# lambdaclass/lambdaworks_kzg

Hardware: NVIDIA B200
Metric: blobs/sec commit+proof (higher is better)
Workload: dtype u32 (12x32-bit Montgomery limbs, IMAD.WIDE)

## Files before the change

### lambdaworks_kzg_b200/csrc/kernels.h

```cpp
#pragma once
#include <cuda_runtime.h>
#include <stddef.h>
#include <stdint.h>

#define LW_SAME_CARVEOUT(kernel)                                                                              \
  do {                                                                                                        \
    static bool lw_done_[64] = {};                                                                            \
    int lw_dev_ = 0;                                                                                          \
    if (cudaGetDevice(&lw_dev_) == cudaSuccess && lw_dev_ >= 0 && lw_dev_ < 64 && !lw_done_[lw_dev_]) {       \
      cudaFuncSetAttribute(kernel, cudaFuncAttributePreferredSharedMemoryCarveout, cudaSharedmemCarveoutMaxShared); \
      lw_done_[lw_dev_] = true;                                                                               \
    }                                                                                                         \
  } while (0)

namespace lw {

constexpr int N_POINTS = 4096;
constexpr int BLOB_BYTES = 4096 * 32;
constexpr int AFFINE_BYTES = 96;
constexpr int XYZZ_BYTES = 192;

uint64_t launches();
void count_launch(int n = 1);

void launch_srs_import(void* d_aff_out, const void* d_canon_in, int* d_not_on_curve, int* d_not_in_subgroup, int n, cudaStream_t st);
void launch_table_bases(void* d_bases, const void* d_aff, int c, int nwin, int npoints, cudaStream_t st);
void launch_table_fill(void* d_table, const void* d_bases, int c, int nwin, int npoints, uint32_t cnt_top, cudaStream_t st);
int table_num_windows(int c);
uint32_t table_top_count(int c);
unsigned long long table_entries(int c, int npoints);

void launch_msm_gather(void* d_partials, const void* d_table, int c, const void* d_scalars, bool be_input,
                       int n_blobs, int blocks_per_blob, cudaStream_t st);
void launch_msm_gather_ba(void* d_partials, const void* d_table, int c, const void* d_scalars, bool be_input,
                          int n_blobs, void* d_scratch, cudaStream_t st, int split = 1);
size_t msm_ba_scratch_bytes(int n_blobs);
int msm_ba_threads();
int msm_ba_slots();
int msm_ba_num_variants();
void msm_ba_set_variant(int v);
void launch_msm_finalize(void* d_out48, void* d_aff_out, const void* d_partials, int parts_per_blob, int n_blobs, cudaStream_t st);
int msm_threads_per_block();

void launch_challenge_midstate(void* d_states, const void* d_blobs, int n, cudaStream_t st, bool latency = false, bool be_header = false);
void launch_challenge_finish(void* d_z, const void* d_states, const void* d_blobs, const void* d_commit48, int n, cudaStream_t st, bool le_digest = false);
void launch_fr_from_be(void* d_z, const void* d_z_be32, int n, cudaStream_t st);
void launch_poly_eval_quot(void* d_q, void* d_y, void* d_y_be32, const void* d_blobs, const void* d_z, int n, cudaStream_t st);

void launch_g1_decompress(void* d_aff, void* d_recompressed48, int* d_status, const void* d_in48, int n, cudaStream_t st, bool strict = false,
                          bool check_subgroup = true);
void launch_g1_subgroup_check(int* d_status, const void* d_aff, int n, cudaStream_t st, bool strict = false);
void launch_status_or(int* d_status, const int* d_other, int n, cudaStream_t st);
void launch_zero_failed(void* d_out, int bytes_per_item, const int* d_status, int n, cudaStream_t st);

void launch_synth_blobs(void* d_blobs, uint64_t first_blob, size_t n, cudaStream_t st);
double run_imad_peak(int variant);

struct G2PreparedDev;
size_t g2_prepared_bytes();
void launch_g2_prepare(void* d_prepared, int* d_bad, const void* d_canon_in, cudaStream_t st);
void launch_g2_check(int* d_bad, const void* d_canon_in, int n, cudaStream_t st);
void launch_verify_single(int* d_ok, const void* d_c_aff, const void* d_pi_aff, const void* d_z, const void* d_y,
                          const void* d_g1_0_aff, const void* d_prep0, const void* d_prep1, bool g1_0_in_subgroup, cudaStream_t st,
                          int* d_status = nullptr, int sub_code = 0);
void launch_make_tuples(void* d_tuples160, const void* d_c48, const void* d_z, const void* d_y, const void* d_pi48, int n, cudaStream_t st, bool le = false);
void launch_batch_challenge(void* d_r, const void* d_tuples160, size_t n_total, cudaStream_t st, int wire = 0);
size_t batch_challenge_state_bytes();
int batch_challenge_blocks_ready(size_t tuples_ready);
void launch_batch_challenge_part(void* d_r, void* d_state, const void* d_tuples160, size_t n_total, int blk0, int blk1, bool first, bool last,
                                 cudaStream_t st, int wire = 0);
void launch_batch_partials(void* d_partial288, const void* d_r, const void* d_c_aff, const void* d_pi_aff, const void* d_z, const void* d_y,
                           size_t first, int n_local, void* d_scratch, cudaStream_t st, cudaStream_t st2, cudaEvent_t ev_fork, cudaEvent_t ev_join);
size_t batch_partials_scratch_bytes(int n_local);
void launch_batch_final(int* d_ok, const void* d_partials288, int n_ranks, const void* d_prep0, const void* d_prep1, cudaStream_t st);
void launch_batch_final_each(int* d_ok, const void* d_partials288, int n_checks, const void* d_prep0, const void* d_prep1, cudaStream_t st);

void launch_write_generator(void* d_out, cudaStream_t st);
void launch_le_roots(void* d_roots, cudaStream_t st);
void launch_le_idft_rows(void* d_rows, cudaStream_t st);
void launch_affine_to_canon(void* d_out24, const void* d_aff, int n, cudaStream_t st);
void launch_le_blob_check(int* d_status, const void* d_blobs, int n, cudaStream_t st, bool be = false);
void launch_le_fr_parse(void* d_out, int* d_status, const void* d_in32, int n, cudaStream_t st, bool be = false);
void launch_le_eval_quot(void* d_q, void* d_y, void* d_y_le32, const void* d_blobs, const void* d_z, const void* d_roots, int n, cudaStream_t st,
                         bool be = false);

void launch_var_msm(void* d_out48, const void* d_points_xy_be, const void* d_scalars_be, size_t n, void* d_scratch, cudaStream_t st,
                    bool points_in_g1 = false);
void launch_var_msm_mont(void* d_out_affine_be96, const void* d_points_mont, const void* d_scalars_canon8, size_t n, void* d_scratch, cudaStream_t st);
size_t var_msm_scratch_bytes(size_t n);
size_t var_msm_bad_flag_offset(size_t n, bool points_in_g1 = false);
int var_msm_window_bits(size_t n);
void launch_var_msm_synth(void* d_pts_be, void* d_sc_be, const void* d_table, unsigned long long n_entries, unsigned long long seed, size_t n,
                          cudaStream_t st);

}
```

### lambdaworks_kzg_b200/csrc/lwkzg.cu

```cuda
#include <cuda_runtime.h>
#include <fcntl.h>
#include <signal.h>
#include <sys/file.h>
#include <unistd.h>

#include <algorithm>
#include <atomic>
#include <condition_variable>
#include <chrono>
#include <cstdio>
#include <cstdlib>
#include <cstring>
#include <map>
#include <mutex>
#include <string>
#include <thread>
#include <vector>

#include "../../include/lwkzg.h"
#include "kernels.h"
#include "kernels_cells.h"
#include "kernels_setup.h"

namespace {
// ... 548 lines not shown
  c->mode = mode;
  c->c = c->nwin = 0;
  c->srs_valid = c->srs_in_g1 = c->g2_valid = false;
  c->g1_host = g1;
  c->g2_host = g2;
  if (!build_ctx_inner(c, g1, g2, mode, window_override)) {
    std::string e = tl_err;
    destroy_ctx(c);
    set_err(e);
    return nullptr;
  }
  return c;
}

struct LazyKey {
  const void* g1;
  const void* g2;
  uint64_t hash;
  bool operator<(const LazyKey& o) const {
    if (g1 != o.g1) return g1 < o.g1;
    if (g2 != o.g2) return g2 < o.g2;
    return hash < o.hash;
  }
};
std::map<LazyKey, Ctx*>& lazy_map() {
  static std::map<LazyKey, Ctx*> m;
  return m;
}
uint64_t fnv1a(const void* p, size_t n, uint64_t h) {
  const uint64_t* w = (const uint64_t*)p;
  for (size_t i = 0; i < n / 8; i++) {
    h ^= w[i];
    h *= 1099511628211ull;
  }
  return h;
}

std::mutex g_lazy_mu;

void destroy_ctx_locked(Ctx* c) {
  if (!c) return;
  { std::lock_guard<std::mutex> lk(c->mu); }
  destroy_ctx(c);
}

Ctx* ctx_of(const KZGSettings* s) {
  if (!s || !s->g1_values || !s->g2_values) {
    set_err("null KZGSettings");
    return nullptr;
  }
  if (s->fs) {
    Ctx* c = reinterpret_cast<Ctx*>(s->fs);
    if (c->magic == CTX_MAGIC) return c;
  }
  LazyKey key{s->g1_values, s->g2_values, 0};
  key.hash = fnv1a(s->g1_values, sizeof(g1_t) * N_POINTS);
  key.hash = fnv1a(s->g2_values, sizeof(g2_t) * 2, key.hash);
  std::lock_guard<std::mutex> lk(g_lazy_mu);
  auto it = lazy_map().find(key);
  if (it != lazy_map().end()) return it->second;
  for (auto j = lazy_map().begin(); j != lazy_map().end();) {
    if (j->first.g1 == key.g1 && j->first.g2 == key.g2) {
      destroy_ctx_locked(j->second);
      j = lazy_map().erase(j);
    } else {
      ++j;
    }
  }
  Ctx* c = build_ctx(s->g1_values, s->g2_values);
  if (c) lazy_map()[key] = c;
  return c;
}

enum class Mode { Commit, CommitProve, BlobProof, PointProof };

bool use_batch_affine(int n) {
  std::lock_guard<std::mutex> lk(g_mu);
  return opts().msm_algo == 1 && n >= opts().msm_ba_min_blobs;
}

size_t chunk_at(size_t off, size_t n, size_t chunk) { return std::min(chunk, n - off); }

int ba_block_slots() {
  static int slots[64] = {};
  int dev = 0;
  if (cudaGetDevice(&dev) != cudaSuccess || dev < 0 || dev >= 64) return 444;
  if (!slots[dev]) {
    int sms = 148;
    cudaDeviceGetAttribute(&sms, cudaDevAttrMultiProcessorCount, dev);
    slots[dev] = 3 * sms;
  }
  return slots[dev];
}

int auto_bpb(int n) {
  if (use_batch_affine(n)) {
    int split = 1;
    while (split < 8 && n * split * 2 <= ba_block_slots()) split *= 2;
    return split;
  }
  long o;
  {
    std::lock_guard<std::mutex> lk(g_mu);
    o = opts().msm_blocks_per_blob;
  }
  if (o > 0) return (int)o;
  int target = (1024 + n - 1) / n;
  int b = 1;
  while (b < target) b <<= 1;
  return std::min(b, 128);
}

void run_msm(Slot& s, const Ctx* c, const void* d_scalars, bool be_input, int n, int bpb, cudaStream_t st);

BufList slot_buffers(Slot& s, int n, int bpb, bool need_blobs) {
  const size_t m = (size_t)n;
  BufList bufs;
  if (use_batch_affine(n)) bufs.push_back({&s.ba_scratch, msm_ba_scratch_bytes(n * bpb)});
  if (need_blobs) bufs.push_back({&s.blobs, m * BLOB_BYTES});
  bufs.insert(bufs.end(), {{&s.q, m * BLOB_BYTES}, {&s.partials, m * bpb * XYZZ_BYTES}, {&s.states, m * 32}, {&s.z, m * 32}, {&s.y, m * 32},
                           {&s.ybe, m * 32}, {&s.c48, m * 48}, {&s.cin48, m * 48}, {&s.p48, m * 48}, {&s.caff, m * AFFINE_BYTES},
                           {&s.status, m * sizeof(int)}, {&s.status2, m * sizeof(int)}, {&s.zbe, m * 32}});
  return bufs;
}

void run_msm(Slot& s, const Ctx* c, const void* d_scalars, bool be_input, int n, int bpb, cudaStream_t st) {
  if (bpb <= 8 && use_batch_affine(n) && s.ba_scratch.cap >= msm_ba_scratch_bytes(n * bpb))
    launch_msm_gather_ba(s.partials.p, c->d_table, c->c, d_scalars, be_input, n, s.ba_scratch.p, st, bpb);
  else
    launch_msm_gather(s.partials.p, c->d_table, c->c, d_scalars, be_input, n, bpb, st);
}

bool enqueue_chunk(Ctx* c, Slot& s, Mode mode, const void* d_blobs, int n, void* d_c48, void* d_p48, void* d_ybe, int* d_status,
                   const void* d_commit_in48, const void* d_z_in_be) {
  const int bpb = auto_bpb(n);
  cudaStream_t st = s.st;
  const bool le = c->lagrange();
  if (le) {
    const bool be = c->be_wire();
    int* stt = d_status ? d_status : (int*)s.status.p;
    CU_TRY(cudaMemsetAsync(stt, 0, (size_t)n * sizeof(int), st));
    launch_le_blob_check(stt, d_blobs, n, st, be);
    if (mode == Mode::Commit) {
      run_msm(s, c, d_blobs, be, n, bpb, st);
      launch_msm_finalize(d_c48, nullptr, s.partials.p, bpb, n, st);
      return true;
    }
    const void* commit_for_hash = nullptr;
    if (mode == Mode::CommitProve || mode == Mode::BlobProof) {
      CU_TRY(cudaEventRecord(s.ev_fork, st));
      CU_TRY(cudaStreamWaitEvent(s.aux, s.ev_fork, 0));
      launch_challenge_midstate(s.states.p, d_blobs, n, s.aux, mode == Mode::BlobProof, be);
      CU_TRY(cudaEventRecord(s.ev_aux, s.aux));
    }
    if (mode == Mode::CommitProve) {
      run_msm(s, c, d_blobs, be, n, bpb, st);
      launch_msm_finalize(d_c48, nullptr, s.partials.p, bpb, n, st);
      commit_for_hash = d_c48;
    } else if (mode == Mode::BlobProof) {
      launch_g1_decompress(nullptr, nullptr, (int*)s.status2.p, d_commit_in48, n, st, true);
      launch_status_or(stt, (const int*)s.status2.p, n, st);
      commit_for_hash = d_commit_in48;
    }
    if (mode == Mode::PointProof) {
      CU_TRY(cudaMemsetAsync(s.status2.p, 0, (size_t)n * sizeof(int), st));
      launch_le_fr_parse(s.z.p, (int*)s.status2.p, d_z_in_be, n, st, be);
      launch_status_or(stt, (const int*)s.status2.p, n, st);
    } else {
      CU_TRY(cudaStreamWaitEvent(st, s.ev_aux, 0));
      launch_challenge_finish(s.z.p, s.states.p, d_blobs, commit_for_hash, n, st, !be);
    }
    launch_le_eval_quot(s.q.p, nullptr, d_ybe, d_blobs, s.z.p, c->d_roots, n, st, be);
    run_msm(s, c, s.q.p, false, n, bpb, st);
    launch_msm_finalize(d_p48, nullptr, s.partials.p, bpb, n, st);
    return true;
// ... 588 lines not shown

bool first_bad_status(Ctx* c, size_t n, int& code) {
  std::vector<int> st(n);
  CU_TRY(cudaMemcpy(st.data(), c->vb_status.p, n * sizeof(int), cudaMemcpyDeviceToHost));
  code = 0;
  for (int v : st)
    if (v) { code = v; break; }
  return true;
}
C_KZG_RET bad_code(int code) { return code == 1 ? C_KZG_BADARGS : C_KZG_ERROR; }

bool verify_single_from_workspace(Ctx* c, bool& ok, bool deferred_subgroup = false, int* bad = nullptr) {
  cudaStream_t s0 = c->slot[0].st;
  launch_verify_single((int*)c->vb_ok.p, c->vb_caff.p, c->vb_piaff.p, c->vb_z.p, c->vb_y.p, c->lagrange() ? c->d_gen : c->d_srs, c->d_prep0, c->d_prep1,
                       c->lagrange() || c->srs_in_g1, s0, deferred_subgroup ? (int*)c->vb_status.p : nullptr, c->lagrange() ? 1 : 2);
  int out[2] = {0, 0};
  CU_TRY(cudaMemcpyAsync(&out[0], c->vb_ok.p, sizeof(int), cudaMemcpyDeviceToHost, s0));
  if (deferred_subgroup) CU_TRY(cudaMemcpyAsync(&out[1], c->vb_status.p, sizeof(int), cudaMemcpyDeviceToHost, s0));
  CU_TRY(cudaStreamSynchronize(s0));
  CU_TRY(cudaGetLastError());
  ok = out[0] != 0;
  if (bad) *bad = out[1];
  return true;
}

struct CtxLock {
  Ctx* c;
  std::unique_lock<std::mutex> lk;
  DeviceGuard dg;
  explicit CtxLock(Ctx* ctx) : c(ctx), lk(ctx->mu), dg(ctx->device) {}
};

#include "cells_host.inl"

}

extern "C" {

const char* lwkzg_last_error(void) { return tl_err.c_str(); }
const char* lwkzg_version(void) { return "lwkzg-b200 0.2 (sm_100a)"; }
uint64_t lwkzg_kernel_launches(void) { return lw::launches(); }

int lwkzg_set_option(const char* name, long value) {
  std::lock_guard<std::mutex> lk(g_mu);
  std::string n(name ? name : "");
  if (n == "window_bits") { if (value < 4 || value > 16) return 1; opts().window_bits = value; return 0; }
  if (n == "msm_blocks_per_blob") { if (value < 0 || value > 256 || (value > 64 && (value & (value - 1)))) return 1; opts().msm_blocks_per_blob = value; return 0; }
  if (n == "chunk_blobs") { if (value < 1 || value > (1 << 20)) return 1; opts().chunk_blobs = value; return 0; }
  if (n == "mode") { if (value < 0 || value > 2) return 1; opts().mode = value; return 0; }
  if (n == "msm_algo") { if (value != 0 && value != 1) return 1; opts().msm_algo = value; return 0; }
  if (n == "msm_ba_min_blobs") { if (value < 1) return 1; opts().msm_ba_min_blobs = value; return 0; }
  if (n == "verify_super_blobs") { if (value < 1) return 1; opts().verify_super_blobs = value; return 0; }
  if (n == "lincomb_points_in_g1") { if (value != 0 && value != 1) return 1; opts().lincomb_points_in_g1 = value; return 0; }
  if (n == "share_table") { if (value != 0 && value != 1) return 1; opts().share_table = value; return 0; }
  if (n == "verify_streams") { if (value < 1 || value > 8) return 1; opts().verify_streams = value; return 0; }
  if (n == "verify_split_subgroup") { if (value != 0 && value != 1) return 1; opts().verify_split_subgroup = value; return 0; }
  if (n == "cache_config") { if (value < 0 || value > 3) return 1; opts().cache_config = value; return 0; }
  if (n == "verify_overlap_decode") { if (value != 0 && value != 1) return 1; opts().verify_overlap_decode = value; return 0; }
  if (n == "cell_window_bits") { if (value < 4 || value > 14) return 1; opts().cell_window_bits = value; return 0; }
  if (n == "cell_chunk_blobs") { if (value < 1 || value > 65536) return 1; opts().cell_chunk_blobs = value; return 0; }
  if (n == "msm_ba_variant") { if (value < 0 || value >= msm_ba_num_variants()) return 1; msm_ba_set_variant((int)value); return 0; }
  return 1;
}
long lwkzg_get_option(const char* name) {
  std::lock_guard<std::mutex> lk(g_mu);
  std::string n(name ? name : "");
  if (n == "window_bits") return opts().window_bits;
  if (n == "msm_blocks_per_blob") return opts().msm_blocks_per_blob;
  if (n == "chunk_blobs") return opts().chunk_blobs;
  if (n == "mode") return opts().mode;
  if (n == "msm_algo") return opts().msm_algo;
  if (n == "msm_ba_min_blobs") return opts().msm_ba_min_blobs;
  if (n == "verify_super_blobs") return opts().verify_super_blobs;
  if (n == "lincomb_points_in_g1") return opts().lincomb_points_in_g1;
  if (n == "share_table") return opts().share_table;
  if (n == "verify_streams") return opts().verify_streams;
  if (n == "verify_split_subgroup") return opts().verify_split_subgroup;
  if (n == "cache_config") return opts().cache_config;
  if (n == "verify_overlap_decode") return opts().verify_overlap_decode;
  if (n == "cell_window_bits") return opts().cell_window_bits;
  if (n == "cell_chunk_blobs") return opts().cell_chunk_blobs;
  if (n == "msm_ba_threads") return msm_ba_threads();
  if (n == "msm_ba_slots") return msm_ba_slots();
  return -1;
}

double lwkzg_imad_peak(int variant) { return lw::run_imad_peak(variant); }

C_KZG_RET load_trusted_setup(KZGSettings* out, const uint8_t* g1_bytes, size_t n1, const uint8_t* g2_bytes, size_t n2) {
  if (n1 != TRUSTED_SETUP_NUM_G1_POINTS || n2 != TRUSTED_SETUP_NUM_G2_POINTS) return C_KZG_BADARGS;
  if (!out || !g1_bytes || !g2_bytes) return C_KZG_ERROR;
  return settings_from_compressed(out, g1_bytes, n1, g2_bytes, n2);
}

C_KZG_RET load_trusted_setup_file(KZGSettings* out, FILE* in) {
  if (!out || !in) return C_KZG_ERROR;
  std::string contents;
  char buf[65536];
  size_t got;
  while ((got = fread(buf, 1, sizeof(buf), in)) > 0) contents.append(buf, got);
  std::vector<std::string> lines;
  size_t pos = 0;
  while (pos < contents.size()) {
    size_t nl = contents.find('\n', pos);
    std::string ln = contents.substr(pos, nl == std::string::npos ? std::string::npos : nl - pos);
    if (!ln.empty() && ln.back() == '\r') ln.pop_back();
    lines.push_back(ln);
    if (nl == std::string::npos) break;
    pos = nl + 1;
  }
  size_t n1 = 0, n2 = 0;
  if (lines.size() < 2 || !parse_usize(lines[0], n1) || !parse_usize(lines[1], n2)) { set_err("invalid trusted setup header"); return C_KZG_ERROR; }
  if (n1 > (1u << 20) || n2 > (1u << 20)) { set_err("implausible point counts"); return C_KZG_ERROR; }
  size_t avail = lines.size() - 2;
  size_t m1 = std::min(n1, avail), m2 = std::min(n2, avail - m1);
  std::vector<uint8_t> g1b(m1 * 48 + 1), g2b(m2 * 96 + 1);
  for (size_t i = 0; i < m1; i++)
    if (!hex_line(lines[2 + i], &g1b[i * 48], 48)) { set_err("bad G1 hex line"); return C_KZG_ERROR; }
  for (size_t i = 0; i < m2; i++)
    if (!hex_line(lines[2 + m1 + i], &g2b[i * 96], 96)) { set_err("bad G2 hex line"); return C_KZG_ERROR; }
  return settings_from_compressed(out, g1b.data(), m1, g2b.data(), m2);
}

C_KZG_RET free_trusted_setup(KZGSettings* s) {
  if (!s) return C_KZG_OK;
  if (s->fs) {
    Ctx* c = reinterpret_cast<Ctx*>(s->fs);
    if (c->magic == CTX_MAGIC) destroy_ctx_locked(c);
    s->fs = nullptr;
  } else {
    std::lock_guard<std::mutex> lk(g_lazy_mu);
    for (auto j = lazy_map().begin(); j != lazy_map().end();) {
      if (j->first.g1 == s->g1_values && j->first.g2 == s->g2_values) {
        destroy_ctx_locked(j->second);
        j = lazy_map().erase(j);
      } else {
        ++j;
      }
    }
  }
  free(s->g1_values);
  free(s->g2_values);
  s->g1_values = nullptr;
  s->g2_values = nullptr;
  return C_KZG_OK;
}

C_KZG_RET lwkzg_blob_to_kzg_commitment_batch(KZGCommitment* out, const Blob* blobs, size_t n, const KZGSettings* s, int* status) {
  return host_batch(Mode::Commit, s, n, blobs, nullptr, nullptr, out, nullptr, nullptr, status);
}
C_KZG_RET lwkzg_compute_blob_kzg_proof_batch(KZGProof* out, const Blob* blobs, const Bytes48* commitments, size_t n, const KZGSettings* s, int* status) {
  return host_batch(Mode::BlobProof, s, n, blobs, commitments, nullptr, nullptr, out, nullptr, status);
}
C_KZG_RET lwkzg_compute_kzg_proof_batch(KZGProof* proofs, Bytes32* ys, const Blob* blobs, const Bytes32* zs, size_t n, const KZGSettings* s, int* status) {
  return host_batch(Mode::PointProof, s, n, blobs, nullptr, zs, nullptr, proofs, ys, status);
}
C_KZG_RET lwkzg_commit_and_prove_batch(KZGCommitment* commitments, KZGProof* proofs, const Blob* blobs, size_t n, const KZGSettings* s, int* status) {
  return host_batch(Mode::CommitProve, s, n, blobs, nullptr, nullptr, commitments, proofs, nullptr, status);
}

C_KZG_RET lwkzg_commit_and_prove_batch_device(void* d_commitments, void* d_proofs, const void* d_blobs, size_t n, const KZGSettings* s, void* stream, void* d_status) {
  return device_batch(Mode::CommitProve, s, n, d_blobs, nullptr, d_commitments, d_proofs, d_status, (cudaStream_t)stream);
}
C_KZG_RET lwkzg_blob_to_kzg_commitment_batch_device(void* d_commitments, const void* d_blobs, size_t n, const KZGSettings* s, void* stream, void* d_status) {
  return device_batch(Mode::Commit, s, n, d_blobs, nullptr, d_commitments, nullptr, d_status, (cudaStream_t)stream);
}
// ... 446 lines not shown
```

### lambdaworks_kzg_b200/csrc/msm.cu

```cuda
#include "msm_common.cuh"

namespace lw {

int msm_threads_per_block() { return MSM_THREADS; }

template <bool BE>
__global__ void __launch_bounds__(MSM_THREADS, LWKZG_MSM_MIN_BLOCKS)
msm_gather_kernel(G1Xyzz* __restrict__ partials, const uint4* __restrict__ table, const uint8_t* __restrict__ scalars,
                  int c, int nwin, uint32_t cnt_top, int pt_threads, int wsplit) {
  constexpr int HT = MSM_THREADS / 2;
  __shared__ uint32_t sk[4][MSM_THREADS];
  __shared__ uint32_t red[48 * HT];

  const int tid = threadIdx.x;
  const int half = tid / HT;
  const int blob = blockIdx.y;
  const int q = blockIdx.x * HT + (tid % HT);
  const int pl = q % pt_threads;
  const int wg = q / pt_threads;
  const uint8_t* sc = scalars + (size_t)blob * BLOB_BYTES;
  auto limb = [&](int w) { return sk[w][tid]; };

  G1Xyzz acc = xyzz_inf();

  for (int pi = pl; pi < N_POINTS; pi += pt_threads) {
    uint32_t h4[4];
    load_scalar_half<BE>(h4, sc, pi, half);
#pragma unroll
    for (int i = 0; i < 4; i++) sk[i][tid] = h4[i];
    int carry = 0;
    int d = 0;
    G1Affine cur = g1a_inf();
    for (int j = 0; j <= nwin; j++) {
      int dn = 0;
      G1Affine nxt = g1a_inf();
      if (j < nwin) {
        dn = glv_digit(limb, c, nwin, j, carry);
        if ((j % wsplit) != wg) dn = 0;
        if (dn != 0) nxt = load_entry(table, entry_index(c, nwin, cnt_top, j, pi, dn < 0 ? -dn : dn));
      }
      if (d != 0) {
        cur.y = fp_cneg(cur.y, d < 0);
        xyzz_madd_hot(acc, cur);
      }
      cur = nxt; d = dn;
    }
  }

  block_reduce_xyzz_glv<MSM_THREADS>(acc, red);
  if (tid == 0) partials[(size_t)blob * gridDim.x + blockIdx.x] = acc;
}

void launch_msm_gather(void* d_partials, const void* d_table, int c, const void* d_scalars, bool be_input, int n_blobs,
                       int blocks_per_blob, cudaStream_t st);
#define LW_BA_DECL(N) void launch_ba_v##N(void*, const void*, int, const void*, bool, int, void*, cudaStream_t, int)
LW_BA_DECL(0); LW_BA_DECL(1);
struct BaVariant { int k, threads; };
static const BaVariant BA_VARIANTS[] = {{64, 128}, {64, 64}};
constexpr int N_BA_VARIANTS = (int)(sizeof(BA_VARIANTS) / sizeof(BA_VARIANTS[0]));
static int g_ba_variant = 0;
void msm_ba_set_variant(int v) { if (v >= 0 && v < N_BA_VARIANTS) g_ba_variant = v; }
int msm_ba_num_variants() { return N_BA_VARIANTS; }
int msm_ba_threads() { return BA_VARIANTS[g_ba_variant].threads; }
int msm_ba_slots() { return BA_VARIANTS[g_ba_variant].k; }
size_t msm_ba_scratch_bytes(int n_blobs) {
  return (size_t)n_blobs * 64 * 9 * 128 * sizeof(uint4);
}

void launch_msm_gather_ba(void* d_partials, const void* d_table, int c, const void* d_scalars, bool be_input, int n_blobs,
                          void* d_scratch, cudaStream_t st, int split) {
  if (n_blobs <= 0) return;
  if (glv_num_windows(c) > BA_VARIANTS[g_ba_variant].k) {
    launch_msm_gather(d_partials, d_table, c, d_scalars, be_input, n_blobs, split, st);
    return;
  }
  switch (g_ba_variant) {
    case 1: launch_ba_v1(d_partials, d_table, c, d_scalars, be_input, n_blobs, d_scratch, st, split); break;
    default: launch_ba_v0(d_partials, d_table, c, d_scalars, be_input, n_blobs, d_scratch, st, split); break;
  }
  count_launch();
}

__global__ void __launch_bounds__(32)
msm_finalize_kernel(uint8_t* __restrict__ out48, G1Affine* __restrict__ aff_out, const G1Xyzz* __restrict__ partials,
                    int parts, int n) {
  const int blob = blockIdx.x * blockDim.x + threadIdx.x;
  if (blob >= n) return;
  const G1Xyzz* p = partials + (size_t)blob * parts;
  G1Xyzz acc = p[0];
  for (int i = 1; i < parts; i++) {
    G1Xyzz o = p[i];
    xyzz_add_ni(acc, o);
  }
  G1Affine a = xyzz_to_affine(acc);
  if (aff_out) aff_out[blob] = a;
  if (out48) g1_compress(out48 + (size_t)blob * 48, a);
}

void launch_msm_gather(void* d_partials, const void* d_table, int c, const void* d_scalars, bool be_input, int n_blobs,
                       int blocks_per_blob, cudaStream_t st) {
  if (n_blobs <= 0) return;
  const int total = blocks_per_blob * (MSM_THREADS / 2);
  const int pt = total < N_POINTS ? total : N_POINTS;
  const int ws = total / pt;
  const int nwin = glv_num_windows(c);
  const uint32_t cnt_top = glv_top_max(c) + 1u;
  for (int b0 = 0; b0 < n_blobs; b0 += 65535) {
    const int nb = n_blobs - b0 < 65535 ? n_blobs - b0 : 65535;
    dim3 grid(blocks_per_blob, nb);
    G1Xyzz* part = (G1Xyzz*)d_partials + (size_t)b0 * blocks_per_blob;
    const uint8_t* sc = (const uint8_t*)d_scalars + (size_t)b0 * BLOB_BYTES;
    if (be_input)
      msm_gather_kernel<true><<<grid, MSM_THREADS, 0, st>>>(part, (const uint4*)d_table, sc, c, nwin, cnt_top, pt, ws);
    else
      msm_gather_kernel<false><<<grid, MSM_THREADS, 0, st>>>(part, (const uint4*)d_table, sc, c, nwin, cnt_top, pt, ws);
  }
  count_launch();
}

__global__ void __launch_bounds__(32) msm_finalize_warp_kernel(uint8_t* __restrict__ out48, G1Affine* __restrict__ aff_out,
                                                                const G1Xyzz* __restrict__ partials, int parts, int n) {
  __shared__ uint32_t red[48 * 16];
  const int blob = blockIdx.x, lane = threadIdx.x;
  const G1Xyzz* p = partials + (size_t)blob * parts;
  G1Xyzz acc = xyzz_inf();
  for (int i = lane; i < parts; i += 32) {
    G1Xyzz o = p[i];
    xyzz_add_ni(acc, o);
  }
  for (int s = 16; s > 0; s >>= 1) {
    if (lane >= s && lane < 2 * s) xyzz_to_smem(red, 16, lane - s, acc);
    __syncwarp();
    if (lane < s) {
      G1Xyzz o = xyzz_from_smem(red, 16, lane);
      xyzz_add_ni(acc, o);
    }
    __syncwarp();
  }
  if (lane == 0) {
    G1Affine a = xyzz_to_affine(acc);
    if (aff_out) aff_out[blob] = a;
    if (out48) g1_compress(out48 + (size_t)blob * 48, a);
  }
}

void launch_msm_finalize(void* d_out48, void* d_aff_out, const void* d_partials, int parts_per_blob, int n_blobs, cudaStream_t st) {
  if (n_blobs <= 0) return;
// ... 9 lines not shown
```

### lambdaworks_kzg_b200/csrc/msm_ba.cuh

```cuda
#pragma once
#include "msm_common.cuh"

namespace lw {

LW_COLD Fp fp_inv_gcd_ni(Fp y) { return fp_inv_gcd(y); }
LW_COLD G1Affine g1a_dbl_ni(G1Affine p) { return xyzz_to_affine(xyzz_dbl_affine(p)); }

#ifndef LWKZG_BA_PREFETCH
#define LWKZG_BA_PREFETCH false
#endif
constexpr uint32_t BA_NONE = 0xffffffffu;

template <int TH>
__device__ __forceinline__ Fp load_fp_scratch(const uint4* p ) {
  uint4 v0 = __ldcg(p), v1 = __ldcg(p + TH), v2 = __ldcg(p + 2 * TH);
  Fp e;
  e.l[0] = v0.x; e.l[1] = v0.y; e.l[2] = v0.z; e.l[3] = v0.w;
  e.l[4] = v1.x; e.l[5] = v1.y; e.l[6] = v1.z; e.l[7] = v1.w;
  e.l[8] = v2.x; e.l[9] = v2.y; e.l[10] = v2.z; e.l[11] = v2.w;
  return e;
}
template <int TH>
__device__ __forceinline__ void store_fp_scratch(uint4* p, const Fp& e) {
  __stcg(p, make_uint4(e.l[0], e.l[1], e.l[2], e.l[3]));
  __stcg(p + TH, make_uint4(e.l[4], e.l[5], e.l[6], e.l[7]));
  __stcg(p + 2 * TH, make_uint4(e.l[8], e.l[9], e.l[10], e.l[11]));
}
__device__ __forceinline__ Fp load_entry_x(const uint4* __restrict__ table, size_t idx) {
  const uint4* p = table + idx * 6;
  uint4 v0 = __ldg(p), v1 = __ldg(p + 1), v2 = __ldg(p + 2);
  Fp e;
  e.l[0] = v0.x; e.l[1] = v0.y; e.l[2] = v0.z; e.l[3] = v0.w;
  e.l[4] = v1.x; e.l[5] = v1.y; e.l[6] = v1.z; e.l[7] = v1.w;
  e.l[8] = v2.x; e.l[9] = v2.y; e.l[10] = v2.z; e.l[11] = v2.w;
  return e;
}

__device__ __forceinline__ void prefetch_l2(const void* p) { asm volatile("prefetch.global.L2 [%0];" ::"l"(p)); }
__device__ __forceinline__ void prefetch_entry_l2(const uint4* table, size_t idx) {
  const uint4* p = table + idx * 6;
  prefetch_l2(p);
  prefetch_l2(p + 4);
}
template <int TH>
__device__ __forceinline__ void prefetch_fp_scratch(const uint4* p) {
  prefetch_l2(p); prefetch_l2(p + TH); prefetch_l2(p + 2 * TH);
}
template <int TH>
__device__ __forceinline__ void prefetch_slot_l2(const uint4* p) {
#pragma unroll
  for (int w = 0; w < 9; w++) prefetch_l2(p + w * TH);
}

__device__ __forceinline__ void cp_async16(uint4* smem_dst, const uint4* gsrc) {
  const uint32_t s = (uint32_t)__cvta_generic_to_shared(smem_dst);
  asm volatile("cp.async.cg.shared.global [%0], [%1], 16;" ::"r"(s), "l"(gsrc) : "memory");
}
__device__ __forceinline__ void cp_async_commit() { asm volatile("cp.async.commit_group;" ::: "memory"); }
__device__ __forceinline__ void cp_async_wait_all() { asm volatile("cp.async.wait_group 0;" ::: "memory"); }
template <int TH>
__device__ __forceinline__ Fp fp_from_stage(const uint4* p ) {
  const uint4 v0 = p[0], v1 = p[TH], v2 = p[2 * TH];
  Fp e;
  e.l[0] = v0.x; e.l[1] = v0.y; e.l[2] = v0.z; e.l[3] = v0.w;
  e.l[4] = v1.x; e.l[5] = v1.y; e.l[6] = v1.z; e.l[7] = v1.w;
  e.l[8] = v2.x; e.l[9] = v2.y; e.l[10] = v2.z; e.l[11] = v2.w;
  return e;
}

template <int TH>
__device__ __forceinline__ void fp_to_stage(uint4* p , const Fp& e) {
  p[0] = make_uint4(e.l[0], e.l[1], e.l[2], e.l[3]);
  p[TH] = make_uint4(e.l[4], e.l[5], e.l[6], e.l[7]);
  p[2 * TH] = make_uint4(e.l[8], e.l[9], e.l[10], e.l[11]);
}

constexpr int BA_STAGE_WORDS = 15;
template <int K, int TH>
constexpr size_t ba_smem_bytes() { return (size_t)BA_STAGE_WORDS * TH * 16 + (size_t)K * TH * 2 + 4 * TH * 4; }

__device__ __forceinline__ uint32_t ba_entry_of(uint32_t code, int c, int nwin, uint32_t cnt_top, int j, int pi) {
  if (code == 0) return BA_NONE;
  int d = (int)code;
  if (j < nwin - 1 && code > 0x8000u) d = (int)code - 65536;
  return entry_index(c, nwin, cnt_top, j, pi, d < 0 ? -d : d) | (d < 0 ? 0x80000000u : 0u);
}

template <bool BE, int K, int TH, bool PF>
__device__ __forceinline__ void msm_gather_ba_body(G1Xyzz* __restrict__ partials, const uint4* __restrict__ table, const uint8_t* __restrict__ scalars,
                                                   uint4* __restrict__ scratch, int c, int nwin, uint32_t cnt_top, int seg_stride, int split) {
  static_assert(K <= 64, "slot masks are 64 bits wide");
  static_assert(48 * (TH / 2) * 4 <= BA_STAGE_WORDS * TH * 16, "the block-reduction scratch aliases the staging area");
  constexpr int HT = TH / 2;
  constexpr int NPT = N_POINTS / HT;
  extern __shared__ uint4 dyn_smem[];
  uint4* stage = dyn_smem + threadIdx.x;
  uint16_t (*sdig)[TH] = reinterpret_cast<uint16_t (*)[TH]>(dyn_smem + BA_STAGE_WORDS * TH);
  uint32_t (*sk)[TH] = reinterpret_cast<uint32_t (*)[TH]>(reinterpret_cast<uint8_t*>(dyn_smem + BA_STAGE_WORDS * TH) + (size_t)K * TH * 2);
  uint32_t* red = reinterpret_cast<uint32_t*>(dyn_smem);

  const int tid = threadIdx.x;
  const int half = tid / HT, hl = tid % HT;
  const int blob = blockIdx.x / split, part = blockIdx.x % split;
  const int npt = NPT / split, p_begin = part * npt;
  const uint8_t* sc = scalars + (size_t)blob * BLOB_BYTES;
  auto limb = [&](int w) { return sk[w][tid]; };
  uint4* my = scratch + (size_t)blockIdx.x * (K * 9 * TH) + tid;

  const int PPR = K / nwin;
  const int rounds = (npt + PPR - 1) / PPR;
  uint64_t infmask = K >= 64 ? ~0ull : ((1ull << K) - 1ull);
  for (int k = PPR * nwin; k < K; k++) sdig[k][tid] = 0;

  auto request1 = [&](int k, uint32_t e) {
    if (e != BA_NONE) {
      const uint4* tp = table + (size_t)(e & 0x7fffffffu) * 6;
      cp_async16(stage, tp); cp_async16(stage + TH, tp + 1); cp_async16(stage + 2 * TH, tp + 2);
      if (!((infmask >> k) & 1ull)) {
        const uint4* ap = my + (k * 9) * TH;
        cp_async16(stage + 6 * TH, ap); cp_async16(stage + 7 * TH, ap + TH); cp_async16(stage + 8 * TH, ap + 2 * TH);
      }
    }
    cp_async_commit();
  };
  auto request2 = [&](int k, uint32_t e) {
    if (e != BA_NONE) {
      const uint4* tp = table + (size_t)(e & 0x7fffffffu) * 6;
#pragma unroll
      for (int w = 0; w < 6; w++) cp_async16(stage + w * TH, tp + w);
      if (!((infmask >> k) & 1ull)) {
        const uint4* ap = my + (k * 9) * TH;
#pragma unroll
        for (int w = 0; w < 9; w++) cp_async16(stage + (6 + w) * TH, ap + w * TH);
      }
    }
    cp_async_commit();
  };

#pragma unroll 1
  for (int rnd = 0; rnd < rounds; rnd++) {
    const int pi0 = hl + HT * (p_begin + rnd * PPR);
#pragma unroll 1
    for (int p = 0; p < PPR; p++) {
      const bool have = rnd * PPR + p < npt;
      const int pi = pi0 + HT * p;
      if (have) {
        uint32_t h4[4];
        load_scalar_half<BE>(h4, sc, pi, half);
#pragma unroll
        for (int i = 0; i < 4; i++) sk[i][tid] = h4[i];
      }
      int carry = 0;
#pragma unroll 1
      for (int j = 0; j < nwin; j++) {
        const int k = p * nwin + j;
        int d = 0;
        if (have) d = glv_digit(limb, c, nwin, j, carry);
        sdig[k][tid] = (uint16_t)d;
        if (PF && d != 0) {
          prefetch_l2(table + (size_t)entry_index(c, nwin, cnt_top, j, pi, d < 0 ? -d : d) * 6);
          if (!((infmask >> k) & 1ull)) prefetch_fp_scratch<TH>(my + (k * 9) * TH);
        }
      }
    }
    Fp prod = fp_one();
    uint64_t specmask = 0;
    uint32_t e_next = ba_entry_of(sdig[0][tid], c, nwin, cnt_top, 0, pi0);
    request1(0, e_next);
    int jn = 0, pin = pi0;
#pragma unroll 1
    for (int k = 0; k < K; k++) {
      const uint32_t e = e_next;
      cp_async_wait_all();
      const bool inf = (infmask >> k) & 1ull;
      Fp d = fp_zero();
      bool tx_zero = false;
      if (e != BA_NONE) {
        const Fp tx = fp_from_stage<TH>(stage);
        tx_zero = fp_is_zero(tx);
        if (!inf) d = fp_sub(tx, fp_from_stage<TH>(stage + 6 * TH));
      }
      if (k + 1 < K) {
        if (++jn == nwin) { jn = 0; pin += HT; }
        e_next = ba_entry_of(sdig[k + 1][tid], c, nwin, cnt_top, jn, pin);
        request1(k + 1, e_next);
      }
      if (e == BA_NONE) continue;
      if (tx_zero) {
        const G1Affine t = load_entry(table, e & 0x7fffffffu);
        if (fp_is_zero(t.y)) { sdig[k][tid] = 0; continue; }
      }
      if (inf) continue;
      if (fp_is_zero(d)) {
        specmask |= 1ull << k;
      } else {
        store_fp_scratch<TH>(my + (k * 9 + 6) * TH, prod);
        prod = fp_mul_nv(prod, d);
      }
    }
    Fp inv = fp_inv_gcd_ni(prod);
    jn = (K - 1) % nwin;
    pin = pi0 + HT * ((K - 1) / nwin);
    e_next = ba_entry_of(sdig[K - 1][tid], c, nwin, cnt_top, jn, pin);
    request2(K - 1, e_next);
#pragma unroll 1
    for (int k = K - 1; k >= 0; k--) {
      const uint32_t e = e_next;
      if (k > 0) {
        if (--jn < 0) { jn = nwin - 1; pin -= HT; }
        e_next = ba_entry_of(sdig[k - 1][tid], c, nwin, cnt_top, jn, pin);
      }
      cp_async_wait_all();
      if (e == BA_NONE) {
        if (k > 0) request2(k - 1, e_next);
        continue;
      }
      G1Affine t;
      t.x = fp_from_stage<TH>(stage);
      t.y = fp_cneg(fp_from_stage<TH>(stage + 3 * TH), (e >> 31) != 0);
      uint4* slot = my + (k * 9) * TH;
      if ((infmask >> k) & 1ull) {
        store_fp_scratch<TH>(slot, t.x);
        store_fp_scratch<TH>(slot + 3 * TH, t.y);
        infmask &= ~(1ull << k);
        if (k > 0) request2(k - 1, e_next);
        continue;
      }
      const Fp ax = fp_from_stage<TH>(stage + 6 * TH), ay = fp_from_stage<TH>(stage + 9 * TH);
      if ((specmask >> k) & 1ull) {
        if (fp_eq(t.y, ay)) {
          const G1Affine dd = g1a_dbl_ni(t);
          store_fp_scratch<TH>(slot, dd.x);
          store_fp_scratch<TH>(slot + 3 * TH, dd.y);
        } else {
          infmask |= 1ull << k;
        }
        if (k > 0) request2(k - 1, e_next);
        continue;
      }
      const Fp d = fp_sub(t.x, ax);
      const Fp dy = fp_sub(t.y, ay);
      const Fp dinv = fp_mul_nv(inv, fp_from_stage<TH>(stage + 12 * TH));
      if (k > 0) request2(k - 1, e_next);
      const Fp lam = fp_mul_nv(dy, dinv);
      inv = fp_mul_nv(inv, d);
      const Fp x3 = fp_sub(fp_sub(fp_sqr_nv(lam), ax), t.x);
      const Fp y3 = fp_sub(fp_mul_nv(lam, fp_sub(ax, x3)), ay);
      store_fp_scratch<TH>(slot, x3);
      store_fp_scratch<TH>(slot + 3 * TH, y3);
    }
  }

  cp_async_wait_all();
  bool acc_inf = true;
#pragma unroll 1
  for (int k = 0; k < K; k++) {
    if ((infmask >> k) & 1ull) continue;
    const Fp px = load_fp_scratch<TH>(my + (k * 9) * TH), py = load_fp_scratch<TH>(my + (k * 9 + 3) * TH);
    if (acc_inf) {
      const Fp one = fp_one();
      fp_to_stage<TH>(stage, px); fp_to_stage<TH>(stage + 3 * TH, py); fp_to_stage<TH>(stage + 6 * TH, one); fp_to_stage<TH>(stage + 9 * TH, one);
      acc_inf = false;
      continue;
    }
    const Fp Pd = fp_sub(fp_mul_nv(px, fp_from_stage<TH>(stage + 6 * TH)), fp_from_stage<TH>(stage));
    const Fp Rd = fp_sub(fp_mul_nv(py, fp_from_stage<TH>(stage + 9 * TH)), fp_from_stage<TH>(stage + 3 * TH));
    if (fp_is_zero(Pd)) {
      G1Xyzz a4;
      a4.x = fp_from_stage<TH>(stage); a4.y = fp_from_stage<TH>(stage + 3 * TH); a4.zz = fp_from_stage<TH>(stage + 6 * TH); a4.zzz = fp_from_stage<TH>(stage + 9 * TH);
      G1Affine p;
      p.x = px; p.y = py;
      xyzz_madd_rare(a4, p);
      if (xyzz_is_inf(a4)) {
        acc_inf = true;
      } else {
        fp_to_stage<TH>(stage, a4.x); fp_to_stage<TH>(stage + 3 * TH, a4.y); fp_to_stage<TH>(stage + 6 * TH, a4.zz); fp_to_stage<TH>(stage + 9 * TH, a4.zzz);
      }
      continue;
    }
    const Fp PP = fp_sqr_nv(Pd), PPP = fp_mul_nv(Pd, PP);
    const Fp Q = fp_mul_nv(fp_from_stage<TH>(stage), PP);
    const Fp X3 = fp_sub(fp_sub(fp_sqr_nv(Rd), PPP), fp_dbl(Q));
    fp_to_stage<TH>(stage, X3);
    const Fp Y3 = fp_sub(fp_mul_nv(Rd, fp_sub(Q, X3)), fp_mul_nv(fp_from_stage<TH>(stage + 3 * TH), PPP));
    fp_to_stage<TH>(stage + 3 * TH, Y3);
    fp_to_stage<TH>(stage + 6 * TH, fp_mul_nv(fp_from_stage<TH>(stage + 6 * TH), PP));
    fp_to_stage<TH>(stage + 9 * TH, fp_mul_nv(fp_from_stage<TH>(stage + 9 * TH), PPP));
  }
  G1Xyzz acc = xyzz_inf();
  if (!acc_inf) {
    acc.x = fp_from_stage<TH>(stage); acc.y = fp_from_stage<TH>(stage + 3 * TH); acc.zz = fp_from_stage<TH>(stage + 6 * TH); acc.zzz = fp_from_stage<TH>(stage + 9 * TH);
  }
  __syncthreads();
  if (seg_stride > 0) {
    if (half == 1) xyzz_to_smem(red, HT, hl, acc);
    __syncthreads();
    if (half == 0) {
      G1Xyzz o = xyzz_from_smem(red, HT, hl);
      xyzz_psi_ni(o);
      xyzz_add_ni(acc, o);
      partials[(size_t)hl * seg_stride + blob] = acc;
    }
    return;
  }
  block_reduce_xyzz_glv<TH>(acc, red);
  if (tid == 0) partials[blockIdx.x] = acc;
}

template <bool BE, int K, int MINB, int TH, bool PF>
__global__ void __launch_bounds__(TH, MINB)
msm_gather_ba_kernel(G1Xyzz* __restrict__ partials, const uint4* __restrict__ table, const uint8_t* __restrict__ scalars,
                     uint4* __restrict__ scratch, int c, int nwin, uint32_t cnt_top, int seg_stride, int split) {
  msm_gather_ba_body<BE, K, TH, PF>(partials, table, scalars, scratch, c, nwin, cnt_top, seg_stride, split);
}
template <bool BE, int K, int REGS, int TH, bool PF>
__global__ void __maxnreg__(REGS)
msm_gather_ba_kernel_r(G1Xyzz* __restrict__ partials, const uint4* __restrict__ table, const uint8_t* __restrict__ scalars,
                       uint4* __restrict__ scratch, int c, int nwin, uint32_t cnt_top, int seg_stride, int split) {
  msm_gather_ba_body<BE, K, TH, PF>(partials, table, scalars, scratch, c, nwin, cnt_top, seg_stride, split);
}

template <int K, int MINB, int TH>
static void launch_ba(void* d_partials, const void* d_table, int c, const void* d_scalars, bool be_input, int n_blobs,
                      void* d_scratch, cudaStream_t st, int seg_stride = 0, int split = 1) {
  const int nwin = glv_num_windows(c);
  const uint32_t cnt_top = glv_top_max(c) + 1u;
  constexpr size_t smem = ba_smem_bytes<K, TH>();
  static bool attr_set = false;
  void (*kbe)(G1Xyzz*, const uint4*, const uint8_t*, uint4*, int, int, uint32_t, int, int);
  void (*kle)(G1Xyzz*, const uint4*, const uint8_t*, uint4*, int, int, uint32_t, int, int);
  if constexpr (MINB > 0) {
    kbe = msm_gather_ba_kernel<true, K, MINB, TH, LWKZG_BA_PREFETCH>;
    kle = msm_gather_ba_kernel<false, K, MINB, TH, LWKZG_BA_PREFETCH>;
  } else {
    kbe = msm_gather_ba_kernel_r<true, K, -MINB, TH, LWKZG_BA_PREFETCH>;
    kle = msm_gather_ba_kernel_r<false, K, -MINB, TH, LWKZG_BA_PREFETCH>;
  }
  if (!attr_set) {
    cudaFuncSetAttribute(kbe, cudaFuncAttributeMaxDynamicSharedMemorySize, (int)smem);
    cudaFuncSetAttribute(kle, cudaFuncAttributeMaxDynamicSharedMemorySize, (int)smem);
    cudaFuncSetAttribute(kbe, cudaFuncAttributePreferredSharedMemoryCarveout, cudaSharedmemCarveoutMaxShared);
    cudaFuncSetAttribute(kle, cudaFuncAttributePreferredSharedMemoryCarveout, cudaSharedmemCarveoutMaxShared);
    attr_set = true;
  }
  if (be_input)
    kbe<<<n_blobs * split, TH, smem, st>>>((G1Xyzz*)d_partials, (const uint4*)d_table, (const uint8_t*)d_scalars, (uint4*)d_scratch, c, nwin, cnt_top, seg_stride, split);
  else
    kle<<<n_blobs * split, TH, smem, st>>>((G1Xyzz*)d_partials, (const uint4*)d_table, (const uint8_t*)d_scalars, (uint4*)d_scratch, c, nwin, cnt_top, seg_stride, split);
}

}
```

### lambdaworks_kzg_b200/csrc/msm_ba_v0.cu

```cuda
#include "msm_ba.cuh"
namespace lw {
void launch_ba_v0(void* d_partials, const void* d_table, int c, const void* d_scalars, bool be_input, int n_blobs, void* d_scratch, cudaStream_t st, int split) {
  launch_ba<64, 3, 128>(d_partials, d_table, c, d_scalars, be_input, n_blobs, d_scratch, st, 0, split);
}
void launch_ba_segmented(void* d_out, const void* d_table, int c, const void* d_scalars, int n_blobs, void* d_scratch, int seg_stride, cudaStream_t st) {
  launch_ba<64, 3, 128>(d_out, d_table, c, d_scalars, false, n_blobs, d_scratch, st, seg_stride);
}
}
```

### lambdaworks_kzg_b200/csrc/msm_ba_v1.cu

```cuda
#include "msm_ba.cuh"
namespace lw {
void launch_ba_v1(void* d_partials, const void* d_table, int c, const void* d_scalars, bool be_input, int n_blobs, void* d_scratch, cudaStream_t st, int split) {
  launch_ba<64, 6, 64>(d_partials, d_table, c, d_scalars, be_input, n_blobs, d_scratch, st, 0, split);
}
}
```

Baseline: 27070.

## Skip batch inversion in first bucket round and size slots by occupancy

```diff
diff --git a/lambdaworks_kzg_b200/csrc/kernels.h b/lambdaworks_kzg_b200/csrc/kernels.h
--- a/lambdaworks_kzg_b200/csrc/kernels.h
+++ b/lambdaworks_kzg_b200/csrc/kernels.h
@@ -37,6 +37,7 @@
 size_t msm_ba_scratch_bytes(int n_blobs);
 int msm_ba_threads();
 int msm_ba_slots();
+int msm_ba_blocks_per_sm();
 int msm_ba_num_variants();
 void msm_ba_set_variant(int v);
 void launch_msm_finalize(void* d_out48, void* d_aff_out, const void* d_partials, int parts_per_blob, int n_blobs, cudaStream_t st);
diff --git a/lambdaworks_kzg_b200/csrc/lwkzg.cu b/lambdaworks_kzg_b200/csrc/lwkzg.cu
--- a/lambdaworks_kzg_b200/csrc/lwkzg.cu
+++ b/lambdaworks_kzg_b200/csrc/lwkzg.cu
@@ -654,15 +654,11 @@
 size_t chunk_at(size_t off, size_t n, size_t chunk) { return std::min(chunk, n - off); }
 
 int ba_block_slots() {
-  static int slots[64] = {};
+  static int sms[64] = {};
   int dev = 0;
   if (cudaGetDevice(&dev) != cudaSuccess || dev < 0 || dev >= 64) return 444;
-  if (!slots[dev]) {
-    int sms = 148;
-    cudaDeviceGetAttribute(&sms, cudaDevAttrMultiProcessorCount, dev);
-    slots[dev] = 3 * sms;
-  }
-  return slots[dev];
+  if (!sms[dev] && cudaDeviceGetAttribute(&sms[dev], cudaDevAttrMultiProcessorCount, dev) != cudaSuccess) sms[dev] = 148;
+  return std::max(1, msm_ba_blocks_per_sm()) * sms[dev];
 }
 
 int auto_bpb(int n) {
@@ -1417,6 +1413,7 @@
   if (n == "cell_chunk_blobs") return opts().cell_chunk_blobs;
   if (n == "msm_ba_threads") return msm_ba_threads();
   if (n == "msm_ba_slots") return msm_ba_slots();
+  if (n == "msm_ba_blocks_per_sm") return msm_ba_blocks_per_sm();
   return -1;
 }
 
diff --git a/lambdaworks_kzg_b200/csrc/msm.cu b/lambdaworks_kzg_b200/csrc/msm.cu
--- a/lambdaworks_kzg_b200/csrc/msm.cu
+++ b/lambdaworks_kzg_b200/csrc/msm.cu
@@ -53,7 +53,7 @@
 
 void launch_msm_gather(void* d_partials, const void* d_table, int c, const void* d_scalars, bool be_input, int n_blobs,
                        int blocks_per_blob, cudaStream_t st);
-#define LW_BA_DECL(N) void launch_ba_v##N(void*, const void*, int, const void*, bool, int, void*, cudaStream_t, int)
+#define LW_BA_DECL(N) void launch_ba_v##N(void*, const void*, int, const void*, bool, int, void*, cudaStream_t, int); int blocks_per_sm_ba_v##N()
 LW_BA_DECL(0); LW_BA_DECL(1);
 struct BaVariant { int k, threads; };
 static const BaVariant BA_VARIANTS[] = {{64, 128}, {64, 64}};
@@ -63,6 +63,7 @@
 int msm_ba_num_variants() { return N_BA_VARIANTS; }
 int msm_ba_threads() { return BA_VARIANTS[g_ba_variant].threads; }
 int msm_ba_slots() { return BA_VARIANTS[g_ba_variant].k; }
+int msm_ba_blocks_per_sm() { return g_ba_variant == 1 ? blocks_per_sm_ba_v1() : blocks_per_sm_ba_v0(); }
 size_t msm_ba_scratch_bytes(int n_blobs) {
   return (size_t)n_blobs * 64 * 9 * 128 * sizeof(uint4);
 }
diff --git a/lambdaworks_kzg_b200/csrc/msm_ba.cuh b/lambdaworks_kzg_b200/csrc/msm_ba.cuh
--- a/lambdaworks_kzg_b200/csrc/msm_ba.cuh
+++ b/lambdaworks_kzg_b200/csrc/msm_ba.cuh
@@ -10,6 +10,27 @@
 #define LWKZG_BA_PREFETCH false
 #endif
 constexpr uint32_t BA_NONE = 0xffffffffu;
+constexpr int BA_INIT_SLOTS = 2;
+
+#ifdef LWKZG_BA_PHASE_PROBE
+constexpr int BA_PROBE_EVENTS = 64;
+enum : uint32_t { BA_PROBE_ENTRY = 1, BA_PROBE_INV = 2, BA_PROBE_EXIT = 3 };
+static __device__ uint4* g_ba_probe;
+__device__ __forceinline__ void ba_probe(int& n, uint32_t kind, int rnd) {
+  uint4* buf = g_ba_probe;
+  if (!buf || (threadIdx.x & 31) != 0 || n >= BA_PROBE_EVENTS) return;
+  uint64_t t;
+  uint32_t sm, wid;
+  asm volatile("mov.u64 %0, %%globaltimer;" : "=l"(t));
+  asm volatile("mov.u32 %0, %%smid;" : "=r"(sm));
+  asm volatile("mov.u32 %0, %%warpid;" : "=r"(wid));
+  const size_t w = (size_t)blockIdx.x * (blockDim.x / 32) + threadIdx.x / 32;
+  buf[w * BA_PROBE_EVENTS + n++] = make_uint4((uint32_t)t, (uint32_t)(t >> 32), sm | (wid << 16), kind | ((uint32_t)rnd << 8));
+}
+#define BA_PROBE(n, kind, rnd) ba_probe(n, kind, rnd)
+#else
+#define BA_PROBE(n, kind, rnd) ((void)(n))
+#endif
 
 template <int TH>
 __device__ __forceinline__ Fp load_fp_scratch(const uint4* p ) {
@@ -90,6 +111,7 @@
 __device__ __forceinline__ void msm_gather_ba_body(G1Xyzz* __restrict__ partials, const uint4* __restrict__ table, const uint8_t* __restrict__ scalars,
                                                    uint4* __restrict__ scratch, int c, int nwin, uint32_t cnt_top, int seg_stride, int split) {
   static_assert(K <= 64, "slot masks are 64 bits wide");
+  static_assert(K % BA_INIT_SLOTS == 0 && 6 * BA_INIT_SLOTS <= BA_STAGE_WORDS, "first round: BA_INIT_SLOTS entries at a time in the staging column");
   static_assert(48 * (TH / 2) * 4 <= BA_STAGE_WORDS * TH * 16, "the block-reduction scratch aliases the staging area");
   constexpr int HT = TH / 2;
   constexpr int NPT = N_POINTS / HT;
@@ -101,6 +123,8 @@
 
   const int tid = threadIdx.x;
   const int half = tid / HT, hl = tid % HT;
+  int probe_n = 0;
+  BA_PROBE(probe_n, BA_PROBE_ENTRY, 0);
   const int blob = blockIdx.x / split, part = blockIdx.x % split;
   const int npt = NPT / split, p_begin = part * npt;
   const uint8_t* sc = scalars + (size_t)blob * BLOB_BYTES;
@@ -162,6 +186,36 @@
           if (!((infmask >> k) & 1ull)) prefetch_fp_scratch<TH>(my + (k * 9) * TH);
         }
       }
+    }
+    if (rnd == 0) {
+      int jn = 0, pin = pi0;
+#pragma unroll 1
+      for (int k0 = 0; k0 < K; k0 += BA_INIT_SLOTS) {
+        uint32_t e[BA_INIT_SLOTS];
+#pragma unroll
+        for (int i = 0; i < BA_INIT_SLOTS; i++) {
+          e[i] = ba_entry_of(sdig[k0 + i][tid], c, nwin, cnt_top, jn, pin);
+          if (++jn == nwin) { jn = 0; pin += HT; }
+          if (e[i] != BA_NONE) {
+            const uint4* tp = table + (size_t)(e[i] & 0x7fffffffu) * 6;
+#pragma unroll
+            for (int w = 0; w < 6; w++) cp_async16(stage + (6 * i + w) * TH, tp + w);
+          }
+        }
+        cp_async_commit();
+        cp_async_wait_all();
+#pragma unroll
+        for (int i = 0; i < BA_INIT_SLOTS; i++) {
+          if (e[i] == BA_NONE) continue;
+          const Fp tx = fp_from_stage<TH>(stage + 6 * i * TH), ty = fp_from_stage<TH>(stage + (6 * i + 3) * TH);
+          if (fp_is_zero(tx) && fp_is_zero(ty)) continue;
+          uint4* slot = my + ((k0 + i) * 9) * TH;
+          store_fp_scratch<TH>(slot, tx);
+          store_fp_scratch<TH>(slot + 3 * TH, fp_cneg(ty, (e[i] >> 31) != 0));
+          infmask &= ~(1ull << (k0 + i));
+        }
+      }
+      continue;
     }
     Fp prod = fp_one();
     uint64_t specmask = 0;
@@ -198,6 +252,7 @@
         prod = fp_mul_nv(prod, d);
       }
     }
+    BA_PROBE(probe_n, BA_PROBE_INV, rnd);
     Fp inv = fp_inv_gcd_ni(prod);
     jn = (K - 1) % nwin;
     pin = pi0 + HT * ((K - 1) / nwin);
@@ -301,10 +356,12 @@
       xyzz_add_ni(acc, o);
       partials[(size_t)hl * seg_stride + blob] = acc;
     }
+    BA_PROBE(probe_n, BA_PROBE_EXIT, rounds);
     return;
   }
   block_reduce_xyzz_glv<TH>(acc, red);
   if (tid == 0) partials[blockIdx.x] = acc;
+  BA_PROBE(probe_n, BA_PROBE_EXIT, rounds);
 }
 
 template <bool BE, int K, int MINB, int TH, bool PF>
@@ -320,33 +377,43 @@
   msm_gather_ba_body<BE, K, TH, PF>(partials, table, scalars, scratch, c, nwin, cnt_top, seg_stride, split);
 }
 
+using BaKernel = void (*)(G1Xyzz*, const uint4*, const uint8_t*, uint4*, int, int, uint32_t, int, int);
+template <int K, int MINB, int TH>
+static BaKernel ba_kernel(bool be) {
+  if constexpr (MINB > 0)
+    return be ? msm_gather_ba_kernel<true, K, MINB, TH, LWKZG_BA_PREFETCH> : msm_gather_ba_kernel<false, K, MINB, TH, LWKZG_BA_PREFETCH>;
+  else
+    return be ? msm_gather_ba_kernel_r<true, K, -MINB, TH, LWKZG_BA_PREFETCH> : msm_gather_ba_kernel_r<false, K, -MINB, TH, LWKZG_BA_PREFETCH>;
+}
+
+template <int K, int MINB, int TH>
+static void ba_set_attributes() {
+  static bool done[64] = {};
+  int dev = 0;
+  if (cudaGetDevice(&dev) != cudaSuccess || dev < 0 || dev >= 64 || done[dev]) return;
+  for (bool be : {true, false}) {
+    cudaFuncSetAttribute(ba_kernel<K, MINB, TH>(be), cudaFuncAttributeMaxDynamicSharedMemorySize, (int)ba_smem_bytes<K, TH>());
+    cudaFuncSetAttribute(ba_kernel<K, MINB, TH>(be), cudaFuncAttributePreferredSharedMemoryCarveout, cudaSharedmemCarveoutMaxShared);
+  }
+  done[dev] = true;
+}
+
+template <int K, int MINB, int TH>
+static int ba_blocks_per_sm() {
+  ba_set_attributes<K, MINB, TH>();
+  int b = 0;
+  if (cudaOccupancyMaxActiveBlocksPerMultiprocessor(&b, ba_kernel<K, MINB, TH>(false), TH, ba_smem_bytes<K, TH>()) != cudaSuccess) return 0;
+  return b;
+}
+
 template <int K, int MINB, int TH>
 static void launch_ba(void* d_partials, const void* d_table, int c, const void* d_scalars, bool be_input, int n_blobs,
                       void* d_scratch, cudaStream_t st, int seg_stride = 0, int split = 1) {
   const int nwin = glv_num_windows(c);
   const uint32_t cnt_top = glv_top_max(c) + 1u;
-  constexpr size_t smem = ba_smem_bytes<K, TH>();
-  static bool attr_set = false;
-  void (*kbe)(G1Xyzz*, const uint4*, const uint8_t*, uint4*, int, int, uint32_t, int, int);
-  void (*kle)(G1Xyzz*, const uint4*, const uint8_t*, uint4*, int, int, uint32_t, int, int);
-  if constexpr (MINB > 0) {
-    kbe = msm_gather_ba_kernel<true, K, MINB, TH, LWKZG_BA_PREFETCH>;
-    kle = msm_gather_ba_kernel<false, K, MINB, TH, LWKZG_BA_PREFETCH>;
-  } else {
-    kbe = msm_gather_ba_kernel_r<true, K, -MINB, TH, LWKZG_BA_PREFETCH>;
-    kle = msm_gather_ba_kernel_r<false, K, -MINB, TH, LWKZG_BA_PREFETCH>;
-  }
-  if (!attr_set) {
-    cudaFuncSetAttribute(kbe, cudaFuncAttributeMaxDynamicSharedMemorySize, (int)smem);
-    cudaFuncSetAttribute(kle, cudaFuncAttributeMaxDynamicSharedMemorySize, (int)smem);
-    cudaFuncSetAttribute(kbe, cudaFuncAttributePreferredSharedMemoryCarveout, cudaSharedmemCarveoutMaxShared);
-    cudaFuncSetAttribute(kle, cudaFuncAttributePreferredSharedMemoryCarveout, cudaSharedmemCarveoutMaxShared);
-    attr_set = true;
-  }
-  if (be_input)
-    kbe<<<n_blobs * split, TH, smem, st>>>((G1Xyzz*)d_partials, (const uint4*)d_table, (const uint8_t*)d_scalars, (uint4*)d_scratch, c, nwin, cnt_top, seg_stride, split);
-  else
-    kle<<<n_blobs * split, TH, smem, st>>>((G1Xyzz*)d_partials, (const uint4*)d_table, (const uint8_t*)d_scalars, (uint4*)d_scratch, c, nwin, cnt_top, seg_stride, split);
-}
-
-}
+  ba_set_attributes<K, MINB, TH>();
+  ba_kernel<K, MINB, TH>(be_input)<<<n_blobs * split, TH, ba_smem_bytes<K, TH>(), st>>>((G1Xyzz*)d_partials, (const uint4*)d_table, (const uint8_t*)d_scalars,
+                                                                                   (uint4*)d_scratch, c, nwin, cnt_top, seg_stride, split);
+}
+
+}
diff --git a/lambdaworks_kzg_b200/csrc/msm_ba_v0.cu b/lambdaworks_kzg_b200/csrc/msm_ba_v0.cu
--- a/lambdaworks_kzg_b200/csrc/msm_ba_v0.cu
+++ b/lambdaworks_kzg_b200/csrc/msm_ba_v0.cu
@@ -3,7 +3,14 @@
 void launch_ba_v0(void* d_partials, const void* d_table, int c, const void* d_scalars, bool be_input, int n_blobs, void* d_scratch, cudaStream_t st, int split) {
   launch_ba<64, 3, 128>(d_partials, d_table, c, d_scalars, be_input, n_blobs, d_scratch, st, 0, split);
 }
+int blocks_per_sm_ba_v0() { return ba_blocks_per_sm<64, 3, 128>(); }
 void launch_ba_segmented(void* d_out, const void* d_table, int c, const void* d_scalars, int n_blobs, void* d_scratch, int seg_stride, cudaStream_t st) {
   launch_ba<64, 3, 128>(d_out, d_table, c, d_scalars, false, n_blobs, d_scratch, st, seg_stride);
 }
 }
+
+#ifdef LWKZG_BA_PHASE_PROBE
+extern "C" int lwkzg_ba_probe_buffer(void* d_buf) {
+  return cudaMemcpyToSymbol(lw::g_ba_probe, &d_buf, sizeof(d_buf)) == cudaSuccess ? 0 : 1;
+}
+#endif
diff --git a/lambdaworks_kzg_b200/csrc/msm_ba_v1.cu b/lambdaworks_kzg_b200/csrc/msm_ba_v1.cu
--- a/lambdaworks_kzg_b200/csrc/msm_ba_v1.cu
+++ b/lambdaworks_kzg_b200/csrc/msm_ba_v1.cu
@@ -3,4 +3,5 @@
 void launch_ba_v1(void* d_partials, const void* d_table, int c, const void* d_scalars, bool be_input, int n_blobs, void* d_scratch, cudaStream_t st, int split) {
   launch_ba<64, 6, 64>(d_partials, d_table, c, d_scalars, be_input, n_blobs, d_scratch, st, 0, split);
 }
+int blocks_per_sm_ba_v1() { return ba_blocks_per_sm<64, 6, 64>(); }
 }
```

New measurement: 27210, median of 6. About the same (+0.5%).
